# irconde/SSL4POLYP

Hardware: AMD Instinct MI355X
Metric: training-step images/sec/node, ViT-B/16 224^2 (cls fine-tune) (higher is better)
Workload: dtype bf16; 1 GPU; ViT-B/16 classification fine-tune, bs=64/GPU, 224^2, AdamW, random init, finetune mode full (finetune.py:49-91); global_batch=64, parallelism=dp1, launch=eager, lr_schedule=constant

## Files before the change

### ssl4polyp_amd/csrc/pm_layernorm.hip

```cpp
#include "pm_common.h"

namespace {

constexpr int kMaxD = 1280;

template <typename TOut, int NV>
__global__ __launch_bounds__(256) void ln_fwd_kernel(const float* __restrict__ x, long ldx, const float* __restrict__ gamma,
                                                     const float* __restrict__ beta, TOut* __restrict__ y,
                                                     float* __restrict__ mean_out, float* __restrict__ rstd_out, int M,
                                                     int D, float eps) {
  constexpr int kMaxVec = NV;
  const int lane = threadIdx.x & 63;
  const int wave = threadIdx.x >> 6;
  const int nvec = D >> 2;
  for (long row = (long)blockIdx.x * 4 + wave; row < M; row += (long)gridDim.x * 4) {
    const float* xr = x + row * ldx;
    f32x4 v[kMaxVec];
    float s = 0.f;
#pragma unroll
    for (int i = 0; i < kMaxVec; ++i) {
      const int c = lane + 64 * i;
      if (c < nvec) {
        v[i] = *reinterpret_cast<const f32x4*>(xr + 4 * c);
        s += (v[i][0] + v[i][1]) + (v[i][2] + v[i][3]);
      }
    }
    const float mean = wave_sum(s) / (float)D;
    float q = 0.f;
#pragma unroll
    for (int i = 0; i < kMaxVec; ++i) {
      const int c = lane + 64 * i;
      if (c < nvec) {
#pragma unroll
        for (int e = 0; e < 4; ++e) {
          const float d = v[i][e] - mean;
          q += d * d;
        }
      }
    }
    const float rstd = rsqrtf(wave_sum(q) / (float)D + eps);
    if (lane == 0) {
      mean_out[row] = mean;
      rstd_out[row] = rstd;
    }
    TOut* yr = y + row * (long)D;
#pragma unroll
    for (int i = 0; i < kMaxVec; ++i) {
      const int c = lane + 64 * i;
      if (c < nvec) {
        const f32x4 g = *reinterpret_cast<const f32x4*>(gamma + 4 * c);
        const f32x4 b = *reinterpret_cast<const f32x4*>(beta + 4 * c);
        f32x4 o;
#pragma unroll
        for (int e = 0; e < 4; ++e) o[e] = (v[i][e] - mean) * rstd * g[e] + b[e];
        store4<TOut>(yr + 4 * c, o);
      }
    }
  }
}

template <typename TDy, typename TAct, int NV>
__global__ __launch_bounds__(256) void ln_bwd_kernel(const TDy* __restrict__ dy, const float* __restrict__ x, long ldx,
                                                     const float* __restrict__ gamma, const float* __restrict__ mean,
                                                     const float* __restrict__ rstd, const float* __restrict__ dres,
                                                     long lddres, float* __restrict__ dx, long lddx,
                                                     TAct* __restrict__ dx_act, float* __restrict__ dgamma,
                                                     float* __restrict__ dbeta, float* __restrict__ dcolsum,
                                                     float* __restrict__ partials, int M, int D) {
  __shared__ float red[3][4][256 + 4];
  constexpr int kMaxVec = NV;
  const int lane = threadIdx.x & 63;
  const int wave = threadIdx.x >> 6;
  const int nvec = D >> 2;
  f32x4 g[kMaxVec];
  f32x4 acc_g[kMaxVec], acc_b[kMaxVec], acc_c[kMaxVec];
#pragma unroll
  for (int i = 0; i < kMaxVec; ++i) {
    const int c = lane + 64 * i;
    const f32x4 z = {0.f, 0.f, 0.f, 0.f};
    g[i] = (c < nvec) ? *reinterpret_cast<const f32x4*>(gamma + 4 * c) : z;
    acc_g[i] = z;
    acc_b[i] = z;
    acc_c[i] = z;
  }
  const float invD = 1.0f / (float)D;
  const long stride = (long)gridDim.x * 4;
  for (long row0 = (long)blockIdx.x * 4 + wave; row0 < M; row0 += 2 * stride) {
    long rows[2] = {row0, row0 + stride};
    const bool valid[2] = {true, rows[1] < M};
    if (!valid[1]) rows[1] = row0;
    float mu[2], rs[2], s1[2] = {0.f, 0.f}, s2[2] = {0.f, 0.f};
    f32x4 xh[2][kMaxVec], dv[2][kMaxVec], dr[2][kMaxVec];
#pragma unroll
    for (int u = 0; u < 2; ++u) {
      mu[u] = mean[rows[u]];
      rs[u] = rstd[rows[u]];
#pragma unroll
      for (int i = 0; i < kMaxVec; ++i) {
        const int c = lane + 64 * i;
        if (c < nvec) {
          xh[u][i] = *reinterpret_cast<const f32x4*>(x + rows[u] * ldx + 4 * c);
          dv[u][i] = load4<TDy>(dy + rows[u] * (long)D + 4 * c);
          if (dres) dr[u][i] = *reinterpret_cast<const f32x4*>(dres + rows[u] * lddres + 4 * c);
        }
      }
    }
#pragma unroll
    for (int u = 0; u < 2; ++u) {
      const float live = valid[u] ? 1.0f : 0.0f;
#pragma unroll
      for (int i = 0; i < kMaxVec; ++i) {
        const int c = lane + 64 * i;
        if (c < nvec) {
#pragma unroll
          for (int e = 0; e < 4; ++e) {
            xh[u][i][e] = (xh[u][i][e] - mu[u]) * rs[u];
            const float gg = dv[u][i][e] * g[i][e];
            s1[u] += gg;
            s2[u] += gg * xh[u][i][e];
            acc_g[i][e] += live * dv[u][i][e] * xh[u][i][e];
            acc_b[i][e] += live * dv[u][i][e];
          }
        }
      }
    }
    float c1[2], c2[2];
#pragma unroll
    for (int u = 0; u < 2; ++u) {
      c1[u] = s1[u];
      c2[u] = s2[u];
    }
#pragma unroll
    for (int o = 32; o > 0; o >>= 1) {
      c1[0] += __shfl_xor(c1[0], o, 64);
      c1[1] += __shfl_xor(c1[1], o, 64);
      c2[0] += __shfl_xor(c2[0], o, 64);
      c2[1] += __shfl_xor(c2[1], o, 64);
    }
#pragma unroll
    for (int u = 0; u < 2; ++u) {
      if (!valid[u]) continue;
      const float k1 = c1[u] * invD, k2 = c2[u] * invD;
#pragma unroll
      for (int i = 0; i < kMaxVec; ++i) {
        const int c = lane + 64 * i;
        if (c < nvec) {
          f32x4 o;
#pragma unroll
          for (int e = 0; e < 4; ++e) o[e] = rs[u] * (dv[u][i][e] * g[i][e] - k1 - xh[u][i][e] * k2);
          if (dres) o += dr[u][i];
          *reinterpret_cast<f32x4*>(dx + rows[u] * lddx + 4 * c) = o;
          if (dx_act) store4<TAct>(dx_act + rows[u] * (long)D + 4 * c, o);
#pragma unroll
          for (int e = 0; e < 4; ++e) acc_c[i][e] += o[e];
        }
      }
    }
  }
#pragma unroll
  for (int i = 0; i < kMaxVec; ++i) {
    const int c = lane + 64 * i;
    __syncthreads();
#pragma unroll
    for (int e = 0; e < 4; ++e) {
      red[0][wave][lane * 4 + e] = acc_g[i][e];
      red[1][wave][lane * 4 + e] = acc_b[i][e];
      red[2][wave][lane * 4 + e] = acc_c[i][e];
    }
    __syncthreads();
    if (wave < 3 && c < nvec) {
      float* dst = wave == 0 ? dgamma : (wave == 1 ? dbeta : dcolsum);
      if (dst) {
        f32x4 t;
#pragma unroll
        for (int e = 0; e < 4; ++e)
          t[e] = (red[wave][0][lane * 4 + e] + red[wave][1][lane * 4 + e]) +
                 (red[wave][2][lane * 4 + e] + red[wave][3][lane * 4 + e]);
        if (partials) {
          *reinterpret_cast<f32x4*>(partials + ((long)blockIdx.x * 3 + wave) * D + 4 * c) = t;
        } else {
#pragma unroll
          for (int e = 0; e < 4; ++e) atomicAdd(dst + 4 * c + e, t[e]);
        }
      }
    }
  }
}

__global__ __launch_bounds__(1024) void ln_bwd_reduce_kernel(const float* __restrict__ partials, float* dgamma, float* dbeta,
                                                             float* dcolsum, int nblocks, int D) {
  __shared__ float red[16][64];
  const int lane = threadIdx.x & 63, rg = threadIdx.x >> 6;
  const int d = blockIdx.x * 64 + lane;
  const int v = blockIdx.y;
  float* dst = v == 0 ? dgamma : (v == 1 ? dbeta : dcolsum);
  if (!dst) return;
  float s0 = 0.f;
  if (d < D) s0 = strided_sum<16>(partials + (long)v * D + d, 3L * D, rg, 16, nblocks);
  red[rg][lane] = s0;
  __syncthreads();
  if (rg == 0 && d < D) {
    float t = 0.f;
#pragma unroll
    for (int g = 0; g < 16; ++g) t += red[g][lane];
    dst[d] += t;
  }
}

inline int ln_grid(int M) {
  int g = (M + 3) / 4;
  return g < 1 ? 1 : (g > 1024 ? 1024 : g);
}

}

extern "C" int pm_layernorm_fwd(const float* x, long ldx, const float* gamma, const float* beta, void* y, int out_dtype,
                                float* mean, float* rstd, int M, int D, float eps, void* stream) {
  if (!x || !gamma || !beta || !y || !mean || !rstd) return PM_EINVAL;
  if (M <= 0 || D <= 0 || D > kMaxD || (D & 3) || (ldx & 3)) return PM_ESHAPE;
  const int grid = (M + 3) / 4 > 4096 ? 4096 : (M + 3) / 4;
#define PM_LN_FWD(TO, NV) \
  hipLaunchKernelGGL((ln_fwd_kernel<TO, NV>), dim3(grid), dim3(256), 0, pm_stream(stream), x, ldx, gamma, beta, (TO*)y, mean, rstd, M, D, eps)
  PM_DISPATCH_ACT(out_dtype, T, {
    if (D <= 1024) PM_LN_FWD(T, 4); else PM_LN_FWD(T, 5);
  });
#undef PM_LN_FWD
  return pm_check_launch();
}

extern "C" int pm_layernorm_bwd(const void* dy, int dy_dtype, const float* x, long ldx, const float* gamma,
                                const float* mean, const float* rstd, const float* dres, long lddres, float* dx,
                                long lddx, void* dx_act, int act_dtype, float* dgamma, float* dbeta, float* dcolsum,
                                int M, int D, void* workspace, size_t ws_bytes, void* stream) {
  if (!dy || !x || !gamma || !mean || !rstd || !dx) return PM_EINVAL;
  if (M <= 0 || D <= 0 || D > kMaxD || (D & 3) || (ldx & 3) || (lddx & 3) || (dres && (lddres & 3))) return PM_ESHAPE;
  if (dx_act && act_dtype != dy_dtype) return PM_EINVAL;
  int grid = (M + 3) / 4;
  float* partials = nullptr;
  const bool want_sums = dgamma || dbeta || dcolsum;
  if (want_sums && workspace && ws_bytes >= (size_t)64 * 3 * D * sizeof(float)) {
    int cap = (int)(ws_bytes / ((size_t)3 * D * sizeof(float)));
    if (cap > 1024) cap = 1024;
    if (grid > cap) grid = cap;
    partials = reinterpret_cast<float*>(workspace);
  } else if (grid > 256) {
    grid = 256;
  }
  if (grid < 1) grid = 1;
  hipStream_t s = pm_stream(stream);
  const int nv = (D + 255) / 256;
#define PM_LN_BWD(TD, NV)                                                                                               \
  hipLaunchKernelGGL((ln_bwd_kernel<TD, TD, NV>), dim3(grid), dim3(256), 0, s, (const TD*)dy, x, ldx, gamma, mean, rstd, \
                     dres, lddres, dx, lddx, (TD*)dx_act, dgamma, dbeta, dcolsum, partials, M, D)
  PM_DISPATCH_ACT(dy_dtype, T, {
    if (nv == 1) PM_LN_BWD(T, 1); else if (nv == 2) PM_LN_BWD(T, 2); else if (nv == 3) PM_LN_BWD(T, 3);
    else if (nv == 4) PM_LN_BWD(T, 4); else PM_LN_BWD(T, 5);
  });
#undef PM_LN_BWD
  if (partials)
    hipLaunchKernelGGL(ln_bwd_reduce_kernel, dim3((D + 63) / 64, 3), dim3(1024), 0, s, partials, dgamma, dbeta, dcolsum, grid, D);
  return pm_check_launch();
}
```

Measured before the change: 6214 images/sec.

## Restructure LayerNorm backward with LDS accumulators, software prefetch, and residual specialization

New measurement: 6298 images/sec (median of 6 runs). +1.4%, better.

```diff
diff --git a/ssl4polyp_amd/csrc/pm_layernorm.hip b/ssl4polyp_amd/csrc/pm_layernorm.hip
--- a/ssl4polyp_amd/csrc/pm_layernorm.hip
+++ b/ssl4polyp_amd/csrc/pm_layernorm.hip
@@ -1,3 +1,4 @@
+#include <stdlib.h>
 #include "pm_common.h"
 
 namespace {
@@ -59,123 +60,119 @@
   }
 }
 
-template <typename TDy, typename TAct, int NV>
-__global__ __launch_bounds__(256) void ln_bwd_kernel(const TDy* __restrict__ dy, const float* __restrict__ x, long ldx,
-                                                     const float* __restrict__ gamma, const float* __restrict__ mean,
-                                                     const float* __restrict__ rstd, const float* __restrict__ dres,
-                                                     long lddres, float* __restrict__ dx, long lddx,
-                                                     TAct* __restrict__ dx_act, float* __restrict__ dgamma,
-                                                     float* __restrict__ dbeta, float* __restrict__ dcolsum,
-                                                     float* __restrict__ partials, int M, int D) {
-  __shared__ float red[3][4][256 + 4];
+template <typename TDy, typename TAct, int NV, bool kRes>
+__global__ __launch_bounds__(256, NV <= 3 ? 4 : 1) void ln_bwd_kernel(const TDy* __restrict__ dy, const float* __restrict__ x, long ldx,
+                                                                      const float* __restrict__ gamma, const float* __restrict__ mean,
+                                                                      const float* __restrict__ rstd, const float* dres, long lddres,
+                                                                      float* dx, long lddx, TAct* __restrict__ dx_act,
+                                                                      float* __restrict__ dgamma, float* __restrict__ dbeta,
+                                                                      float* __restrict__ dcolsum, float* __restrict__ partials,
+                                                                      int M, int D) {
+  __shared__ f32x4 gam[NV * 64];
+  __shared__ f32x4 acc[3][4][NV * 64];
   constexpr int kMaxVec = NV;
+  typedef TDy __attribute__((ext_vector_type(4))) Dy4;
   const int lane = threadIdx.x & 63;
-  const int wave = threadIdx.x >> 6;
+  const int wave = __builtin_amdgcn_readfirstlane(threadIdx.x >> 6);
   const int nvec = D >> 2;
-  f32x4 g[kMaxVec];
-  f32x4 acc_g[kMaxVec], acc_b[kMaxVec], acc_c[kMaxVec];
+  const f32x4 z = {0.f, 0.f, 0.f, 0.f};
+  for (int c = threadIdx.x; c < kMaxVec * 64; c += 256) gam[c] = (c < nvec) ? *reinterpret_cast<const f32x4*>(gamma + 4 * c) : z;
+#pragma unroll
+  for (int i = 0; i < kMaxVec; ++i) {
+    acc[0][wave][lane + 64 * i] = z;
+    acc[1][wave][lane + 64 * i] = z;
+    acc[2][wave][lane + 64 * i] = z;
+  }
+  __syncthreads();
+  const float invD = 1.0f / (float)D;
+  const long stride = (long)gridDim.x * 4;
+  long row = (long)blockIdx.x * 4 + wave;
+  f32x4 nx[kMaxVec], ndr[kMaxVec];
+  Dy4 ndy[kMaxVec];
+  float nmu = 0.f, nrs = 0.f;
+  auto fetch = [&](long r) {
+    nmu = mean[r];
+    nrs = rstd[r];
+#pragma unroll
+    for (int i = 0; i < kMaxVec; ++i) {
+      const int c = lane + 64 * i;
+      if (i < kMaxVec - 1 || c < nvec) {
+        nx[i] = *reinterpret_cast<const f32x4*>(x + r * ldx + 4 * c);
+        ndy[i] = *reinterpret_cast<const Dy4*>(dy + r * (long)D + 4 * c);
+        if (kRes) ndr[i] = *reinterpret_cast<const f32x4*>(dres + r * lddres + 4 * c);
+      }
+    }
+  };
+  if (row < M) fetch(row);
+  while (row < M) {
+    const float mu = nmu, rs = nrs;
+    f32x4 xh[kMaxVec], dr[kMaxVec];
+    Dy4 dv[kMaxVec];
+#pragma unroll
+    for (int i = 0; i < kMaxVec; ++i) {
+      const int c = lane + 64 * i;
+      if (i < kMaxVec - 1 || c < nvec) {
+#pragma unroll
+        for (int e = 0; e < 4; ++e) xh[i][e] = (nx[i][e] - mu) * rs;
+        dv[i] = ndy[i];
+        if (kRes) dr[i] = ndr[i];
+      }
+    }
+    const long next = row + stride;
+    if (next < M) fetch(next);
+    float s1 = 0.f, s2 = 0.f;
+#pragma unroll
+    for (int i = 0; i < kMaxVec; ++i) {
+      const int c = lane + 64 * i;
+      if (i < kMaxVec - 1 || c < nvec) {
+        const f32x4 g = gam[c];
+        f32x4 ag = acc[0][wave][c], ab = acc[1][wave][c];
+#pragma unroll
+        for (int e = 0; e < 4; ++e) {
+          const float d = (float)dv[i][e];
+          const float gg = d * g[e];
+          s1 += gg;
+          s2 += gg * xh[i][e];
+          ag[e] = __builtin_fmaf(d, xh[i][e], ag[e]);
+          ab[e] += d;
+        }
+        acc[0][wave][c] = ag;
+        acc[1][wave][c] = ab;
+      }
+      __builtin_amdgcn_sched_barrier(0);
+    }
+    float c1 = s1, c2 = s2;
+#pragma unroll
+    for (int o = 32; o > 0; o >>= 1) {
+      c1 += __shfl_xor(c1, o, 64);
+      c2 += __shfl_xor(c2, o, 64);
+    }
+    const float k1 = c1 * invD, k2 = c2 * invD;
+#pragma unroll
+    for (int i = 0; i < kMaxVec; ++i) {
+      const int c = lane + 64 * i;
+      if (i < kMaxVec - 1 || c < nvec) {
+        const f32x4 g = gam[c];
+        f32x4 o;
+#pragma unroll
+        for (int e = 0; e < 4; ++e) o[e] = rs * ((float)dv[i][e] * g[e] - k1 - xh[i][e] * k2);
+        if (kRes) o += dr[i];
+        *reinterpret_cast<f32x4*>(dx + row * lddx + 4 * c) = o;
+        if (dx_act) store4<TAct>(dx_act + row * (long)D + 4 * c, o);
+        acc[2][wave][c] += o;
+      }
+      __builtin_amdgcn_sched_barrier(0);
+    }
+    row = next;
+  }
+  __syncthreads();
 #pragma unroll
   for (int i = 0; i < kMaxVec; ++i) {
     const int c = lane + 64 * i;
-    const f32x4 z = {0.f, 0.f, 0.f, 0.f};
-    g[i] = (c < nvec) ? *reinterpret_cast<const f32x4*>(gamma + 4 * c) : z;
-    acc_g[i] = z;
-    acc_b[i] = z;
-    acc_c[i] = z;
-  }
-  const float invD = 1.0f / (float)D;
-  const long stride = (long)gridDim.x * 4;
-  for (long row0 = (long)blockIdx.x * 4 + wave; row0 < M; row0 += 2 * stride) {
-    long rows[2] = {row0, row0 + stride};
-    const bool valid[2] = {true, rows[1] < M};
-    if (!valid[1]) rows[1] = row0;
-    float mu[2], rs[2], s1[2] = {0.f, 0.f}, s2[2] = {0.f, 0.f};
-    f32x4 xh[2][kMaxVec], dv[2][kMaxVec], dr[2][kMaxVec];
-#pragma unroll
-    for (int u = 0; u < 2; ++u) {
-      mu[u] = mean[rows[u]];
-      rs[u] = rstd[rows[u]];
-#pragma unroll
-      for (int i = 0; i < kMaxVec; ++i) {
-        const int c = lane + 64 * i;
-        if (c < nvec) {
-          xh[u][i] = *reinterpret_cast<const f32x4*>(x + rows[u] * ldx + 4 * c);
-          dv[u][i] = load4<TDy>(dy + rows[u] * (long)D + 4 * c);
-          if (dres) dr[u][i] = *reinterpret_cast<const f32x4*>(dres + rows[u] * lddres + 4 * c);
-        }
-      }
-    }
-#pragma unroll
-    for (int u = 0; u < 2; ++u) {
-      const float live = valid[u] ? 1.0f : 0.0f;
-#pragma unroll
-      for (int i = 0; i < kMaxVec; ++i) {
-        const int c = lane + 64 * i;
-        if (c < nvec) {
-#pragma unroll
-          for (int e = 0; e < 4; ++e) {
-            xh[u][i][e] = (xh[u][i][e] - mu[u]) * rs[u];
-            const float gg = dv[u][i][e] * g[i][e];
-            s1[u] += gg;
-            s2[u] += gg * xh[u][i][e];
-            acc_g[i][e] += live * dv[u][i][e] * xh[u][i][e];
-            acc_b[i][e] += live * dv[u][i][e];
-          }
-        }
-      }
-    }
-    float c1[2], c2[2];
-#pragma unroll
-    for (int u = 0; u < 2; ++u) {
-      c1[u] = s1[u];
-      c2[u] = s2[u];
-    }
-#pragma unroll
-    for (int o = 32; o > 0; o >>= 1) {
-      c1[0] += __shfl_xor(c1[0], o, 64);
-      c1[1] += __shfl_xor(c1[1], o, 64);
-      c2[0] += __shfl_xor(c2[0], o, 64);
-      c2[1] += __shfl_xor(c2[1], o, 64);
-    }
-#pragma unroll
-    for (int u = 0; u < 2; ++u) {
-      if (!valid[u]) continue;
-      const float k1 = c1[u] * invD, k2 = c2[u] * invD;
-#pragma unroll
-      for (int i = 0; i < kMaxVec; ++i) {
-        const int c = lane + 64 * i;
-        if (c < nvec) {
-          f32x4 o;
-#pragma unroll
-          for (int e = 0; e < 4; ++e) o[e] = rs[u] * (dv[u][i][e] * g[i][e] - k1 - xh[u][i][e] * k2);
-          if (dres) o += dr[u][i];
-          *reinterpret_cast<f32x4*>(dx + rows[u] * lddx + 4 * c) = o;
-          if (dx_act) store4<TAct>(dx_act + rows[u] * (long)D + 4 * c, o);
-#pragma unroll
-          for (int e = 0; e < 4; ++e) acc_c[i][e] += o[e];
-        }
-      }
-    }
-  }
-#pragma unroll
-  for (int i = 0; i < kMaxVec; ++i) {
-    const int c = lane + 64 * i;
-    __syncthreads();
-#pragma unroll
-    for (int e = 0; e < 4; ++e) {
-      red[0][wave][lane * 4 + e] = acc_g[i][e];
-      red[1][wave][lane * 4 + e] = acc_b[i][e];
-      red[2][wave][lane * 4 + e] = acc_c[i][e];
-    }
-    __syncthreads();
-    if (wave < 3 && c < nvec) {
+    if (wave < 3 && (i < kMaxVec - 1 || c < nvec)) {
       float* dst = wave == 0 ? dgamma : (wave == 1 ? dbeta : dcolsum);
       if (dst) {
-        f32x4 t;
-#pragma unroll
-        for (int e = 0; e < 4; ++e)
-          t[e] = (red[wave][0][lane * 4 + e] + red[wave][1][lane * 4 + e]) +
-                 (red[wave][2][lane * 4 + e] + red[wave][3][lane * 4 + e]);
+        const f32x4 t = (acc[wave][0][c] + acc[wave][1][c]) + (acc[wave][2][c] + acc[wave][3][c]);
         if (partials) {
           *reinterpret_cast<f32x4*>(partials + ((long)blockIdx.x * 3 + wave) * D + 4 * c) = t;
         } else {
@@ -207,11 +204,15 @@
   }
 }
 
-inline int ln_grid(int M) {
-  int g = (M + 3) / 4;
-  return g < 1 ? 1 : (g > 1024 ? 1024 : g);
-}
-
+constexpr int kLnBwdBlocks = 1024;
+int ln_bwd_max_blocks() {
+  static const int v = [] {
+    const char* e = getenv("PM_LN_BWD_BLOCKS");
+    const int n = e && e[0] ? atoi(e) : kLnBwdBlocks;
+    return n < 64 ? 64 : (n > 1024 ? 1024 : n);
+  }();
+  return v;
+}
 }
 
 extern "C" int pm_layernorm_fwd(const float* x, long ldx, const float* gamma, const float* beta, void* y, int out_dtype,
@@ -235,23 +236,26 @@
   if (!dy || !x || !gamma || !mean || !rstd || !dx) return PM_EINVAL;
   if (M <= 0 || D <= 0 || D > kMaxD || (D & 3) || (ldx & 3) || (lddx & 3) || (dres && (lddres & 3))) return PM_ESHAPE;
   if (dx_act && act_dtype != dy_dtype) return PM_EINVAL;
-  int grid = (M + 3) / 4;
+  int cap = 256;
   float* partials = nullptr;
   const bool want_sums = dgamma || dbeta || dcolsum;
   if (want_sums && workspace && ws_bytes >= (size_t)64 * 3 * D * sizeof(float)) {
-    int cap = (int)(ws_bytes / ((size_t)3 * D * sizeof(float)));
-    if (cap > 1024) cap = 1024;
-    if (grid > cap) grid = cap;
+    const size_t fit = ws_bytes / ((size_t)3 * D * sizeof(float));
+    cap = ln_bwd_max_blocks();
+    if ((size_t)cap > fit) cap = (int)fit;
     partials = reinterpret_cast<float*>(workspace);
-  } else if (grid > 256) {
-    grid = 256;
-  }
-  if (grid < 1) grid = 1;
+  } else if (!want_sums) {
+    cap = ln_bwd_max_blocks();
+  }
+  const int grid = (M + 3) / 4 < cap ? (M + 3) / 4 : cap;
   hipStream_t s = pm_stream(stream);
   const int nv = (D + 255) / 256;
 #define PM_LN_BWD(TD, NV)                                                                                               \
-  hipLaunchKernelGGL((ln_bwd_kernel<TD, TD, NV>), dim3(grid), dim3(256), 0, s, (const TD*)dy, x, ldx, gamma, mean, rstd, \
-                     dres, lddres, dx, lddx, (TD*)dx_act, dgamma, dbeta, dcolsum, partials, M, D)
+  do {                                                                                                                   \
+    auto kern = dres ? ln_bwd_kernel<TD, TD, NV, true> : ln_bwd_kernel<TD, TD, NV, false>;                               \
+    hipLaunchKernelGGL(kern, dim3(grid), dim3(256), 0, s, (const TD*)dy, x, ldx, gamma, mean, rstd, dres, lddres, dx, lddx, \
+                       (TD*)dx_act, dgamma, dbeta, dcolsum, partials, M, D);                                             \
+  } while (0)
   PM_DISPATCH_ACT(dy_dtype, T, {
     if (nv == 1) PM_LN_BWD(T, 1); else if (nv == 2) PM_LN_BWD(T, 2); else if (nv == 3) PM_LN_BWD(T, 3);
     else if (nv == 4) PM_LN_BWD(T, 4); else PM_LN_BWD(T, 5);
```
